# zhoupengwei/tloam

Hardware: AMD Instinct MI355X
Metric: gauss_newton_iters_per_sec (higher is better)
Workload: dtype f64

## Files before the change

tloam_amd/csrc/tl_gn.hip:

```cpp
#include <stdlib.h>
#include <string.h>

#include <hip/hip_ext.h>

#include "tl_common.hpp"
#include "tl_finish.hpp"

namespace tl {

struct Acc {
  double v[27];
  double pm;
  int pe;
};

__host__ __device__ constexpr int ut(int i, int j) { return i * 6 - (i * (i - 1)) / 2 + (j - i); }

__device__ __forceinline__ double fast_rcp(double x) {
  double r = __builtin_amdgcn_rcp(x);
  return __builtin_fma(r, __builtin_fma(-x, r, 1.0), r);
}
__device__ __forceinline__ double fast_rsqrt(double x) {
  double y = __builtin_amdgcn_rsq(x);
  const double h = 0.5 * x * y;
// ... 688 lines not shown
}
__device__ __forceinline__ void load_state_words(const GnState* st, GnState* sm) {
  constexpr int kWords = (int)(sizeof(GnState) / 8);
  static_assert(kWords <= 256, "one word per thread");
  if (threadIdx.x < kWords)
    reinterpret_cast<unsigned long long*>(sm)[threadIdx.x] = reinterpret_cast<const unsigned long long*>(st)[threadIdx.x];
}
__device__ __forceinline__ void stop_comm_error(GnState* st) {
  if (threadIdx.x == 0) { st->done = 1; st->comm_error = 1; }
}
__device__ __forceinline__ bool mbox_receive(const MboxView& mb, unsigned long long id, double* out , int count, int lane) {
  const bool ok = mbox_gather(mb, id, out, count, lane);
  if (lane == 0) {
    mb.ctr[0] = id;
    if (!ok) mb.ctr[1] = 1ull;
  }
  return ok;
}
__global__ __launch_bounds__(64) void k_gn_step(GnState* st, const double* __restrict__ in48, unsigned long long* iter_span) {
  __shared__ double tot[kReduceBuf];
  __shared__ double scr[32];
  __shared__ GnState s_in;
  if (threadIdx.x < kReduceBuf) tot[threadIdx.x] = in48[threadIdx.x];
  load_state_lds(st, &s_in, threadIdx.x);
  __syncthreads();
  if (s_in.done) return;
  const bool first = s_in.phase == PH_ITER0;
  gn_consume(st, tot, threadIdx.x, &s_in, scr);
  if (threadIdx.x == 0) iter_span_note(iter_span, first);
}
void launch_gn_step(GnState* st, const double* in48, hipStream_t s, unsigned long long* iter_span) {
  hipLaunchKernelGGL(k_gn_step, dim3(1), dim3(64), 0, s, st, in48, iter_span);
}
__global__ __launch_bounds__(64) void k_gn_step_mbox(GnState* st, MboxView mb, unsigned long long* iter_span) {
  __shared__ double tot[kMboxSlot];
  __shared__ double scr[32];
  __shared__ GnState s_in;
  load_state_lds(st, &s_in, threadIdx.x);
  __syncthreads();
  if (s_in.done) return;
  const bool ok = mbox_receive(mb, mbox_next_id(mb), tot, kReduceBuf, threadIdx.x);
  __syncthreads();
  if (!ok) {
    stop_comm_error(st);
    return;
  }
  const bool first = s_in.phase == PH_ITER0;
  gn_consume(st, tot, threadIdx.x, &s_in, scr);
  if (threadIdx.x == 0) iter_span_note(iter_span, first);
}
void launch_gn_step_mbox(GnState* st, const MboxView& mb, hipStream_t s, unsigned long long* iter_span) {
  hipLaunchKernelGGL(k_gn_step_mbox, dim3(1), dim3(64), 0, s, st, mb, iter_span);
}
__global__ __launch_bounds__(64) void k_mbox_gather_only(double* out48, MboxView mb) {
  __shared__ double tot[kMboxSlot];
  mbox_receive(mb, mbox_next_id(mb), tot, kReduceBuf, threadIdx.x);
  if (threadIdx.x < kReduceBuf) out48[threadIdx.x] = tot[threadIdx.x];
}
void launch_mbox_gather_only(double* out48, const MboxView& mb, hipStream_t s) {
  hipLaunchKernelGGL(k_mbox_gather_only, dim3(1), dim3(64), 0, s, out48, mb);
}
__global__ __launch_bounds__(64) void k_mbox_allreduce(double* buf, int count, MboxView mb) {
  __shared__ double vals[kMboxSlot];
  const int t = threadIdx.x;
  if (t < count) vals[t] = buf[t];
  __syncthreads();
  const unsigned long long id = mbox_next_id(mb);
  mbox_post(mb, id, vals, count, t);
  mbox_receive(mb, id, vals, count, t);
  __syncthreads();
  if (t < count) buf[t] = vals[t];
}
void launch_mbox_allreduce(double* buf, int count, const MboxView& mb, hipStream_t s) {
  hipLaunchKernelGGL(k_mbox_allreduce, dim3(1), dim3(64), 0, s, buf, count, mb);
}

__global__ __launch_bounds__(kRedThreads) void k_reduce_and_step(const double* __restrict__ partials, int rows,
                                                                 GnState* __restrict__ st, unsigned long long* iter_span) {
  __shared__ double lds[8 * 33];
  __shared__ double tot[kReduceBuf];
  __shared__ GnState s_in;
#ifdef TLOAM_STEP_PROFILE
  if (threadIdx.x == 0) st->dbg[0] = (double)__builtin_readcyclecounter();
#endif
  load_state_words(st, &s_in);
#ifdef TLOAM_STEP_PROFILE
  asm volatile("s_waitcnt vmcnt(0)" ::: "memory");
  if (threadIdx.x == 0) st->dbg[7] = (double)__builtin_readcyclecounter();
#endif
  fold_rows<false, 4>(partials, rows, lds, tot);
#ifdef TLOAM_STEP_PROFILE
  if (threadIdx.x == 0) st->dbg[8] = (double)__builtin_readcyclecounter();
#endif
  if (s_in.done) return;
  const bool first = s_in.phase == PH_ITER0;
  if (threadIdx.x < 64) gn_consume(st, tot, threadIdx.x, &s_in, lds );
  if (threadIdx.x == 0) iter_span_note(iter_span, first);
#ifdef TLOAM_STEP_PROFILE
  if (threadIdx.x == 0) st->dbg[6] = (double)__builtin_readcyclecounter();
#endif
}
struct K3Step {
  int* ticket;
  unsigned long long* span;
  unsigned long long* iter_span;
  MboxView mb;
};
template <bool SINGLE, int W = 4>
__global__ __launch_bounds__(64 * W, 2) void k3_sweep_step(const double* __restrict__ seg0, int stride0, int cap0, int unused,
                                                        GnState* __restrict__ st, const int* __restrict__ seg_n,
                                                        double* __restrict__ partials, CorrView cv, K3Step fs) {
  __shared__ double red[W][32];
  __shared__ double s_grp[8 * 33];
  __shared__ double tot[kMboxSlot];
  __shared__ GnState s_in;
  SweepStamps ts;
  sweep_body<SINGLE, W, false>(seg0, stride0, cap0, (unused & 2) != 0 , false, st, seg_n, cv, red,
                               ts, [&] {
    if (fs.span && blockIdx.x == 0 && threadIdx.x == 0)
      __hip_atomic_store(fs.span, (unsigned long long)wall_clock64(), __ATOMIC_RELAXED, __HIP_MEMORY_SCOPE_AGENT);
    load_state_words(st, &s_in);
  }, [&] {
    if (!k3_take_ticket<W>(partials, red, fs.ticket)) return;
    if (fs.span && threadIdx.x == 0) {
      const unsigned long long t1 = wall_clock64();
      const unsigned long long t0 = __hip_atomic_load(fs.span, __ATOMIC_RELAXED, __HIP_MEMORY_SCOPE_AGENT);
      fs.span[1] += t1 - t0;
      fs.span[2] += 1ull;
    }
    fold_rows<true>(partials, (int)gridDim.x, s_grp, tot);
    if (threadIdx.x == 0) __hip_atomic_store(fs.ticket, 0, __ATOMIC_RELAXED, __HIP_MEMORY_SCOPE_AGENT);
    if (threadIdx.x >= 64) return;
    if (fs.mb.nranks > 0) {
      const unsigned long long id = mbox_next_id(fs.mb);
      mbox_post(fs.mb, id, tot, kReduceBuf, (int)threadIdx.x);
      const bool ok = mbox_receive(fs.mb, id, tot, kReduceBuf, (int)threadIdx.x);
      asm volatile("s_waitcnt lgkmcnt(0)" ::: "memory");
      if (!ok) {
        stop_comm_error(st);
        return;
      }
    }
    const bool first = s_in.phase == PH_ITER0;
    gn_consume(st, tot, (int)threadIdx.x, &s_in, s_grp );
    if (threadIdx.x == 0) iter_span_note(fs.iter_span, first);
  });
}
void launch_k3_step(const CorrView& cv, GnState* st, double* partials, int grid, bool single, bool wide, int* ticket, unsigned long long* span,
                    const MboxView* mb_or_null, hipStream_t s, hipEvent_t ev_start, hipEvent_t ev_stop, unsigned long long* iter_span) {
  auto kern = single ? k3_sweep_step<true> : wide ? k3_sweep_step<false, 8> : k3_sweep_step<false>;
  K3Step fs;
  memset(&fs, 0, sizeof(fs));
  fs.ticket = ticket;
  fs.span = span;
  fs.iter_span = iter_span;
  if (mb_or_null) fs.mb = *mb_or_null;
  launch_sweep(kern, grid, wide ? 512 : 256, s, ev_start, ev_stop, cv, 0, st, partials, cv, fs);
}

__global__ __launch_bounds__(256, 1) void k_sweep_step_small(const double* __restrict__ seg0, int stride0, int cap0, int tagged,
                                                             GnState* __restrict__ st, const int* __restrict__ seg_n,
                                                             double* __restrict__ partials, int* __restrict__ ticket,
                                                             CorrView cv, unsigned long long* iter_span) {
  __shared__ double red[4][32];
  __shared__ double s_grp[8 * 33];
  __shared__ double s_rows[kTaggedRows * 28];
  __shared__ double tot[kReduceBuf];
  __shared__ GnState s_in;
  const int lane = threadIdx.x & 63, wave = __builtin_amdgcn_readfirstlane(threadIdx.x >> 6);
  const int gw = blockIdx.x * 4 + wave;
#ifdef TLOAM_STEP_PROFILE
  const unsigned long long c_entry = __builtin_readcyclecounter();
#endif
  ChunkData pre;
  const SingleWork wk = single_work_of(cv, cap0, gw, lane);
  const bool w2 = (tagged & 2) != 0;
  tagged &= 1;
  single_fetch(cv, seg0, stride0, wk, pre, w2);
  {
    constexpr int kWords = (int)(sizeof(GnState) / 8);
    static_assert(kWords <= 256, "one word per thread");
    if (threadIdx.x < kWords)
      reinterpret_cast<unsigned long long*>(&s_in)[threadIdx.x] = reinterpret_cast<const unsigned long long*>(st)[threadIdx.x];
  }
  unsigned long long* const epoch = reinterpret_cast<unsigned long long*>(ticket + 2);
  const unsigned long long epoch0 = *epoch;
  if (st->done) return;
  const Rt T = st->Rt_eval;
#ifdef TLOAM_STEP_PROFILE
  asm volatile("s_waitcnt lgkmcnt(0)" ::: "memory");
  const unsigned long long c_pose = __builtin_readcyclecounter();
#endif
  Acc a;
  sweep_single(cv, seg_n, T, wk, pre, a);
#ifdef TLOAM_STEP_PROFILE
  const unsigned long long c_eval = __builtin_readcyclecounter();
#endif
  const double wtot = wave_reduce_acc(a, lane);
  if ((lane & 1) == 0) red[wave][lane >> 1] = wtot;
  __syncthreads();
#ifdef TLOAM_STEP_PROFILE
  const unsigned long long c_sweep = __builtin_readcyclecounter();
#endif
  if (tagged) {
    k3_post_row_tagged(partials, red, epoch0 + 1ull);
    if (blockIdx.x != 0 || threadIdx.x >= 64) return;
#ifdef TLOAM_STEP_PROFILE
    if (threadIdx.x == 0) {
      st->dbg[7] = (double)c_sweep; st->dbg[0] = (double)__builtin_readcyclecounter();
      st->dbg[8] = (double)c_entry; st->dbg[9] = (double)c_pose; st->dbg[10] = (double)c_eval;
    }
#endif
    const bool ok = poll_fold_tagged(partials, (int)gridDim.x, epoch0 + 1ull, s_rows, tot, (int)threadIdx.x);
    if (threadIdx.x == 0) *epoch = epoch0 + 1ull;
    if (!ok) {
      if (threadIdx.x == 0) { st->done = 1; st->comm_error = 1; }
      return;
    }
  } else {
    if (!k3_take_ticket(partials, red, ticket)) return;
#ifdef TLOAM_STEP_PROFILE
    if (threadIdx.x == 0) { st->dbg[7] = (double)c_sweep; st->dbg[0] = (double)__builtin_readcyclecounter(); }
#endif
    fold_rows<true>(partials, (int)gridDim.x, s_grp, tot);
    if (threadIdx.x == 0) __hip_atomic_store(ticket, 0, __ATOMIC_RELAXED, __HIP_MEMORY_SCOPE_AGENT);
  }
  const bool first = s_in.phase == PH_ITER0;
  if (threadIdx.x < 64) gn_consume(st, tot, threadIdx.x, &s_in, s_grp );
  if (threadIdx.x == 0) iter_span_note(iter_span, first);
#ifdef TLOAM_STEP_PROFILE
  if (threadIdx.x == 0) st->dbg[6] = (double)__builtin_readcyclecounter();
#endif
}
void launch_sweep_step_small(const CorrView& cv, GnState* st, double* partials, int* ticket, int grid, hipStream_t s,
                             unsigned long long* iter_span) {
  launch_sweep(k_sweep_step_small, grid, 256, s, nullptr, nullptr, cv, grid <= kTaggedRows ? 1 : 0 , st, partials, ticket, cv,
               iter_span);
}
#include "tl_prep.hpp"

__device__ __forceinline__ bool weight_out_of_range(const WeightParams& wp, int kind, double c) {
  if (!wp.active[kind]) return false;
  if (c == 0) return false;
  if (c >= wp.th1 || c <= wp.th2) return false;
  if (c < wp.th1 * (1.0 - 1e-9) && c > wp.th2 * (1.0 + 1e-9)) return false;
  const double w = sqrt(wp.noise_bound_sq * wp.mu * (wp.mu + 1) / c) - wp.mu;
  return !(w >= 0.0 && w <= 1.0);
}
constexpr int kExtRowBase = 512;
__device__ __forceinline__ void post_ext_segment(double* __restrict__ partials, int gw, double cs, double bad, int kind, unsigned long long tag,
                                                 int lane, int base_word = kExtRowBase) {
  if (lane >= 8) return;
  unsigned long long wd = 0ull;
  const double cs0 = rdlane(cs, 0), bad0 = rdlane(bad, 0);
  if (lane == 0) wd = (unsigned long long)__double_as_longlong(cs0);
  else if (lane == 1) wd = (unsigned long long)__double_as_longlong(bad0);
  else if (lane == 2) wd = (unsigned long long)(long long)kind;
  const unsigned long long x = xor8(lane < 7 ? seg_word(wd, lane) : 0ull);
  if (lane == 7) wd = check_mix(tag) ^ x;
  __hip_atomic_store(reinterpret_cast<unsigned long long*>(partials) + base_word + (size_t)gw * 8 + lane, wd, __ATOMIC_RELAXED,
                     __HIP_MEMORY_SCOPE_AGENT);
}
__device__ __forceinline__ bool poll_fold_ext(const double* __restrict__ partials, int nwaves, unsigned long long tag, double* s_ext ,
                                              double* fin , int lane, int base_word = kExtRowBase) {
  const bool have = lane >= 1 && lane < nwaves;
  const unsigned long long mtag = check_mix(tag);
  const unsigned long long* p = reinterpret_cast<const unsigned long long*>(partials) + base_word + (size_t)(have ? lane : 1) * 8;
  unsigned long long w[8];
  const unsigned long long t0 = wall_clock64();
  bool ok_all;
  for (unsigned spins = 1;; ++spins) {
#pragma unroll
    for (int i = 0; i < 8; ++i) w[i] = __hip_atomic_load(p + i, __ATOMIC_RELAXED, __HIP_MEMORY_SCOPE_AGENT);
    unsigned long long x = w[7];
#pragma unroll
    for (int i = 0; i < 7; ++i) x ^= seg_word(w[i], i);
    ok_all = __all((!have || x == mtag) ? 1 : 0) != 0;
    if (ok_all) break;
    if ((spins & 63u) == 0 && wall_clock64() - t0 > 100000000ull) break;
    __builtin_amdgcn_s_sleep(1);
  }
  const double cs = have ? __longlong_as_double((long long)w[0]) : 0.0;
  const double bad = have ? __longlong_as_double((long long)w[1]) : 0.0;
  const int kind = have ? (int)(long long)w[2] : -1;
  double t[5];
#pragma unroll
  for (int k = 0; k < 4; ++k) t[k] = kind == k ? cs : 0.0;
  t[4] = bad;
#pragma unroll
  for (int off = 32; off > 0; off >>= 1)
#pragma unroll
    for (int k = 0; k < 5; ++k) t[k] += __shfl_down(t[k], off, 64);
  if (lane == 0) {
#pragma unroll
    for (int k = 0; k < 5; ++k) fin[k] = t[k];
  }
  asm volatile("s_waitcnt lgkmcnt(0)" ::: "memory");
  (void)s_ext;
  return ok_all;
}

__device__ __forceinline__ int finish_by_consumer(GnState* st, GnState* sm , const SolveFinish& F, int oi,
                                                  const double* fin, const int nseg[kKinds], double* sh , int lane,
                                                  bool lead = true) {
  constexpr int kWords = (int)(offsetof(GnState, dbg) / 8);
  const OuterCtl ctl{F.cost_threshold, 1, oi == F.n_iter - 1 ? 1 : 0};
  int next = 4;
  if (!sm->done) {
    if (lane == 0) {
      sm->incomplete = OS_INCOMPLETE;
      sm->stop = 2;
      sm->run_build = sm->run_refresh = 0;
    }
  } else {
    if (lane < 16) {
      double v = 0.0;
      if (lane < 4) v = fin[lane];
      else if (lane < 8) v = (double)(lane == 4 ? nseg[0] : (lane == 5 ? nseg[1] : (lane == 6 ? nseg[2] : nseg[3])));
      else if (lane == 8) v = fin[4];
      sh[lane] = v;
      if (lead) F.sums16[lane] = v;
    }
    asm volatile("s_waitcnt lgkmcnt(0)" ::: "memory");
    publish_and_rearm(sh, sm, lane, ctl);
    asm volatile("s_waitcnt lgkmcnt(0)" ::: "memory");
    next = (sm->stop == 0 && sm->run_build == 0 && sm->run_refresh != 0 && oi + 1 < F.n_iter) ? 3 : 4;
  }
  asm volatile("s_waitcnt lgkmcnt(0)" ::: "memory");
  if (!lead) return next;
  for (int w = lane; w < kWords; w += 64) reinterpret_cast<unsigned long long*>(st)[w] = reinterpret_cast<const unsigned long long*>(sm)[w];
  mirror_wave(sm, F.hm[oi], lane, (sm->stop == 0 && next == 4) ? (int)(sm->incomplete | OS_NEEDS_HOST) : -1);
  if (sm->stop != 0)
    for (int j = oi + 1; j < F.n_iter; ++j) mirror_wave(sm, F.hm[j], lane, (int)OS_SKIPPED);
  return next;
}

constexpr int kAllRowsParity = kTaggedRows * kAccStride;
constexpr int kAllExtBase = 2 * kAllRowsParity;
constexpr int kAllExtParity = 64 * 8;
__device__ __forceinline__ bool next_is_failure(const double* s_msg) {
  asm volatile("s_waitcnt lgkmcnt(0)" ::: "memory");
  return (int)s_msg[12] == 5;
}
__global__ __launch_bounds__(256, 1) void k_solve_all(const double* __restrict__ seg0, int stride0, int cap0, int max_sweeps,
                                                      GnState* __restrict__ st, const int* __restrict__ seg_n,
                                                      double* __restrict__ partials, int* __restrict__ ticket, CorrView cv, SolvePrep prep,
                                                      int* __restrict__ seg_n_out, SolveFinish F) {
  __shared__ double red[4][32];
  __shared__ double s_scr[32];
  __shared__ double s_rows[kTaggedRows * 28];
  __shared__ double s_ext[64 * 3];
  __shared__ double s_fin[8];
  __shared__ double s_sh[16];
  __shared__ double tot[kReduceBuf];
  __shared__ double s_msg[16];
  __shared__ GnState s_in;
  const int lane = threadIdx.x & 63, wave = __builtin_amdgcn_readfirstlane(threadIdx.x >> 6);
  const int gw = blockIdx.x * 4 + wave;
  const bool stepper = wave == 0;
  const bool lead = blockIdx.x == 0;
  const bool self_prep = prep.sv.flagb != nullptr;
  const unsigned long long sabotage = ((max_sweeps >> 16) & 1) ? (1ull << 40) : 0ull;
  max_sweeps &= 0xffff;
  unsigned long long* const epoch = reinterpret_cast<unsigned long long*>(ticket + 2);
#ifdef TLOAM_STEP_PROFILE
  unsigned long long* const prof = reinterpret_cast<unsigned long long*>(partials) + 2048;
  const bool prof_c = lead && stepper && lane == 0;
  const bool prof_p = (int)blockIdx.x == (int)gridDim.x / 2 && wave == 1 && lane == 0;
#define TL_PROF(cond, slot) if (cond) prof[(slot)] = wall_clock64();
#else
#define TL_PROF(cond, slot)
#endif
  ChunkData pre;
  const SingleWork wk = single_work_of(cv, cap0, gw, lane);
  single_fetch(cv, seg0, stride0, wk, pre);
  FlagBytes fbytes;
  if (self_prep && wk.kind >= 0) load_flag_bytes(prep.sv.flagb, wk.kind, lane, fbytes);
  if (stepper) {
    constexpr int kWords = (int)(sizeof(GnState) / 8);
    for (int w = lane; w < kWords; w += 64)
      reinterpret_cast<unsigned long long*>(&s_in)[w] = reinterpret_cast<const unsigned long long*>(st)[w];
  }
  const unsigned long long tag0 = (*epoch + 1ull) << 8;
  int oi = F.first_iter;
  if (F.enabled && (st->stop != 0 || st->next_outer != oi)) return;
  const bool build = self_prep && (!prep.run_build || *prep.run_build != 0);
  const bool refresh = self_prep && !build && prep.run_refresh && *prep.run_refresh != 0;
  const bool done_at_entry = st->done != 0;
  Rt T = st->Rt_eval;
  int n_mine = 0;
  int slot[2] = {0, 0};
  int nseg[kKinds] = {0, 0, 0, 0};
  if (lead && stepper) {
    if (build) {
      FlagBytes fb[kKinds];
#pragma unroll
      for (int k = 0; k < kKinds; ++k) load_flag_bytes(prep.sv.flagb, k, lane, fb[k]);
#pragma unroll
      for (int k = 0; k < kKinds; ++k) nseg[k] = kind_set_of(prep, cv, k, lane, fb[k]).total;
      if (lane < kKinds) seg_n_out[lane] = lane == 0 ? nseg[0] : (lane == 1 ? nseg[1] : (lane == 2 ? nseg[2] : nseg[3]));
    } else {
#pragma unroll
      for (int k = 0; k < kKinds; ++k) nseg[k] = seg_n[k];
    }
  }
  if (wk.kind >= 0) {
    if (build) {
      n_mine = self_compact(prep, cv, wk, lane, fbytes, pre, slot);
    } else {
      n_mine = seg_n[wk.kind];
      if (self_prep) {
        slots_of_chunk(prep, cv, wk, n_mine, slot);
        if (refresh) self_refresh(prep, cv, wk, n_mine, slot, pre);
      }
    }
  }
  if (stepper) {
    asm volatile("s_waitcnt vmcnt(0) lgkmcnt(0)" ::: "memory");
    if (build && lane < 6) {
      s_in.x_build[lane] = s_in.x[lane];
      if (lead) st->x_build[lane] = s_in.x[lane];
    }
  }
  if (done_at_entry) return;
  TL_PROF(prof_c, 0)
  unsigned long long h = 0;
  for (;;) {
    int verdict = 2;
    double2 last_cost = double2{0.0, 0.0};
    for (int it = 0;; ++it) {
      Acc a;
      last_cost = double2{0.0, 0.0};
      sweep_single_n(cv, n_mine, T, wk, pre, a, &last_cost);
      TL_PROF(prof_p, 64 + it * 8 + 1)
      const double wtot = wave_reduce_acc(a, lane);
      if ((lane & 1) == 0) red[wave][lane >> 1] = wtot;
      __syncthreads();
      double* const rows = partials + (size_t)(h & 1ull) * kAllRowsParity;
      const int ext_base = kAllExtBase + (int)(h & 1ull) * kAllExtParity;
      k3_post_row_tagged(rows, red, tag0 | h);
      TL_PROF(prof_c, 8 + it * 8 + 0)
      if (F.have_wp) {
        double cs = last_cost.x + last_cost.y;
        double bad = 0.0;
        if (wk.kind >= 0) {
          const bool two = single_chunk_of(wk.kind) == kChunk;
          if (wk.j < n_mine && weight_out_of_range(F.wp[oi], wk.kind, last_cost.x)) bad += 1.0;
          if (two && wk.j + 1 < n_mine && weight_out_of_range(F.wp[oi], wk.kind, last_cost.y)) bad += 1.0;
        }
#pragma unroll
        for (int off = 32; off > 0; off >>= 1) {
          cs += __shfl_down(cs, off, 64);
          bad += __shfl_down(bad, off, 64);
        }
        post_ext_segment(partials, gw, cs, bad, wk.kind, tag0 | h, lane, ext_base);
      }
      TL_PROF(prof_p, 64 + it * 8 + 2)
      if (stepper) {
        const bool ok = poll_fold_tagged(rows, (int)gridDim.x, (tag0 | h) ^ sabotage, s_rows, tot, lane);
        TL_PROF(prof_c, 8 + it * 8 + 1)
        int vd = 5;
        if (ok) {
          gn_consume(st, tot, lane, &s_in, s_scr, false);
          vd = (s_in.done == 0 && it + 1 < max_sweeps) ? 1 : 2;
          if (lead && lane == 0) iter_span_note(F.iter_span, it == 0);
        }
        TL_PROF(prof_c, 8 + it * 8 + 2)
        if (lane < 9) s_msg[lane] = s_in.Rt_eval.r[lane];
        else if (lane < 12) s_msg[lane] = s_in.Rt_eval.t[lane - 9];
        else if (lane == 12) s_msg[12] = (double)vd;
      }
      __syncthreads();
      verdict = (int)s_msg[12];
      if (lead && stepper && verdict != 5) gn_write_back(st, &s_in, lane);
#pragma unroll
      for (int v = 0; v < 9; ++v) T.r[v] = s_msg[v];
#pragma unroll
      for (int v = 0; v < 3; ++v) T.t[v] = s_msg[9 + v];
      TL_PROF(prof_c, 8 + it * 8 + 3)
      TL_PROF(prof_p, 64 + (it + 1) * 8 + 0)
      h += 1ull;
      if (verdict != 1) break;
    }
    if (verdict == 5) {
      if (lead && stepper) {
        if (lane == 0) {
          st->done = 1; st->comm_error = 1;
          s_in.done = 1; s_in.comm_error = 1;
          if (F.enabled) {
            s_in.incomplete = OS_COMM_ERROR;
            st->incomplete = OS_COMM_ERROR;
            st->stop = 1; st->run_build = 0; st->run_refresh = 0;
          }
          *epoch = tag0 >> 8;
        }
        asm volatile("s_waitcnt lgkmcnt(0)" ::: "memory");
        if (F.enabled) {
          mirror_wave(&s_in, F.hm[oi], lane, (int)OS_COMM_ERROR);
          for (int j = oi + 1; j < F.n_iter; ++j) mirror_wave(&s_in, F.hm[j], lane, (int)OS_SKIPPED);
        }
      }
      return;
    }
    double2 w_new = pre.w;
    if (F.enabled && wk.kind >= 0) {
      const bool two = single_chunk_of(wk.kind) == kChunk;
      if (wk.j < n_mine) w_new.x = refreshed_weight(F.wp[oi], wk.kind, last_cost.x, pre.w.x, prep.sv.w_src, slot[0]);
      if (two && wk.j + 1 < n_mine) w_new.y = refreshed_weight(F.wp[oi], wk.kind, last_cost.y, pre.w.y, prep.sv.w_src, slot[1]);
    }
    if (stepper) {
      int next = 4;
      bool ok = true;
      if (F.have_wp)
        ok = poll_fold_ext(partials, (int)gridDim.x * 4, tag0 | (h - 1ull), s_ext, s_fin, lane, kAllExtBase + (int)((h - 1ull) & 1ull) * kAllExtParity);
      if (!ok) {
        next = 5;
      } else if (!F.enabled) {
        if (lead) {
          if (F.have_wp && lane < 5) {
            const double v = s_fin[lane];
            if (lane < 4) st->fin_sum[lane] = v; else st->fin_bad = v;
          }
          if (lane == 0) { st->fin_valid = F.have_wp ? 1 : 0; *epoch = tag0 >> 8; }
        }
      } else {
        next = finish_by_consumer(st, &s_in, F, oi, s_fin, nseg, s_sh, lane, lead);
      }
      if (lane < 9) s_msg[lane] = s_in.Rt_eval.r[lane];
      else if (lane < 12) s_msg[lane] = s_in.Rt_eval.t[lane - 9];
      else if (lane == 12) s_msg[12] = (double)next;
    }
    if (!F.enabled) {
      if (lead && stepper && next_is_failure(s_msg) && lane == 0) {
        st->done = 1; st->comm_error = 1; s_in.done = 1; s_in.comm_error = 1;
        st->fin_valid = 0;
        *epoch = tag0 >> 8;
      }
      return;
    }
    __syncthreads();
    const int next = (int)s_msg[12];
#pragma unroll
    for (int v = 0; v < 9; ++v) T.r[v] = s_msg[v];
#pragma unroll
    for (int v = 0; v < 3; ++v) T.t[v] = s_msg[9 + v];
    if (next == 5) {
      if (lead && stepper) {
        if (lane == 0) {
          st->done = 1; st->comm_error = 1; s_in.done = 1; s_in.comm_error = 1;
          s_in.incomplete = OS_COMM_ERROR; st->incomplete = OS_COMM_ERROR;
          st->stop = 1; st->run_build = 0; st->run_refresh = 0;
          *epoch = tag0 >> 8;
        }
        asm volatile("s_waitcnt lgkmcnt(0)" ::: "memory");
        mirror_wave(&s_in, F.hm[oi], lane, (int)OS_COMM_ERROR);
        for (int j = oi + 1; j < F.n_iter; ++j) mirror_wave(&s_in, F.hm[j], lane, (int)OS_SKIPPED);
      }
      return;
    }
    if (next != 3) {
      if (lead && stepper && lane == 0) *epoch = tag0 >> 8;
      return;
    }
    if (wk.kind >= 0) {
      const CorrSeg& seg = cv.k[wk.kind];
      const bool two = single_chunk_of(wk.kind) == kChunk;
      pre.w = w_new;
      if (wk.j < n_mine) { seg.w[wk.j] = w_new.x; seg.cost[wk.j] = 0.0; }
      if (two && wk.j + 1 < n_mine) { seg.w[wk.j + 1] = w_new.y; seg.cost[wk.j + 1] = 0.0; }
    }
    oi += 1;
  }
}
void launch_solve_small(const CorrView& cv, GnState* st, double* partials, int* ticket, int grid, int max_sweeps,
                        const SolvePrep* prep_or_null, int* seg_n, const SolveFinish* finish_or_null, hipStream_t s) {
  SolvePrep P;
  if (prep_or_null) P = *prep_or_null;
  else memset(&P, 0, sizeof(P));
  SolveFinish F;
  if (finish_or_null) F = *finish_or_null;
  else memset(&F, 0, sizeof(F));
  hipLaunchKernelGGL(k_solve_all, dim3(grid), dim3(256), 0, s, (const double*)cv.k[0].px, cv.k[0].stride, cv.k[0].cap, max_sweeps, st,
                     cv.seg_n, partials, ticket, cv, P, seg_n, F);
}
bool solve_small_fits(int grid, int device_cus) { return grid <= kTaggedRows && grid <= device_cus; }
void launch_reduce_and_step(const double* partials, int grid, GnState* st, hipStream_t s, unsigned long long* iter_span) {
  hipLaunchKernelGGL(k_reduce_and_step, dim3(1), dim3(kRedThreads), 0, s, partials, grid, st, iter_span);
}

__global__ void k_debug_se3(const double* __restrict__ x, const double* __restrict__ delta, int n, double* __restrict__ out) {
  const int i = blockIdx.x * blockDim.x + threadIdx.x;
  if (i >= n) return;
  double xv[6], dv[6];
#pragma unroll
  for (int k = 0; k < 6; ++k) { xv[k] = x[6 * i + k]; dv[k] = delta[6 * i + k]; }
  const Pose E = exp_fast2(dv);
  const Pose X = exp_fast2(xv);
  double lx[6], pl[6];
  log_fast2(X, lx);
  log_fast2(compose_fast2(E, X), pl);
  const Pose X2 = se3_exp(xv);
  double* o = out + 26 * (size_t)i;
  o[0] = E.qw; o[1] = E.qx; o[2] = E.qy; o[3] = E.qz; o[4] = E.tx; o[5] = E.ty; o[6] = E.tz;
#pragma unroll
  for (int k = 0; k < 6; ++k) { o[7 + k] = lx[k]; o[13 + k] = pl[k]; }
  o[19] = X2.qw; o[20] = X2.qx; o[21] = X2.qy; o[22] = X2.qz; o[23] = X2.tx; o[24] = X2.ty; o[25] = X2.tz;
}
void launch_debug_se3(const double* x, const double* delta, int n, double* out, hipStream_t s) {
  hipLaunchKernelGGL(k_debug_se3, dim3((n + 63) / 64), dim3(64), 0, s, x, delta, n, out);
}

__global__ __launch_bounds__(256) void k_weights(WeightArgs A, double* __restrict__ partial, const GnState* __restrict__ st) {
  __shared__ double red[4][8];
  if (!st->done || st->stop) return;
  double sum[kKinds] = {0, 0, 0, 0};
  double bad = 0.0;
  const int tid = blockIdx.x * 256 + threadIdx.x, stride = gridDim.x * 256;
#pragma unroll
  for (int k = 0; k < kKinds; ++k) {
    const int n = A.cv.seg_n[k];
    const CorrSeg& seg = A.cv.k[k];
    constexpr int kU = 4;
    for (int i0 = tid; i0 < n; i0 += kU * stride) {
      double cu[kU];
      int iu[kU];
#pragma unroll
      for (int u = 0; u < kU; ++u) {
        const int i = i0 + u * stride;
        cu[u] = (i < n) ? seg.cost[i] : 0.0;
        iu[u] = (i < n) ? seg.idx[i] : 0;
      }
#pragma unroll
      for (int u = 0; u < kU; ++u) {
        if (i0 + u * stride >= n) break;
        const double c = cu[u];
        sum[k] += c;
        if (!A.wp.active[k]) continue;
        if (c == 0) continue;
        double w;
        if (c >= A.wp.th1) w = 0.0;
        else if (c <= A.wp.th2) w = 1.0;
        else {
          w = sqrt(A.wp.noise_bound_sq * A.wp.mu * (A.wp.mu + 1) / c) - A.wp.mu;
          if (!(w >= 0.0 && w <= 1.0)) bad += 1.0;
        }
        const int slot = A.sv.slot_off[k] + (iu[u] - A.sv.src_lo[k]);
        A.sv.w_src[slot] = w;
      }
    }
  }
  double v[5] = {sum[0], sum[1], sum[2], sum[3], bad};
  const int lane = threadIdx.x & 63, wave = threadIdx.x >> 6;
#pragma unroll
  for (int i = 0; i < 5; ++i) {
#pragma unroll
    for (int off = 32; off > 0; off >>= 1) v[i] += __shfl_down(v[i], off, 64);
    if (lane == 0) red[wave][i] = v[i];
  }
  __syncthreads();
  if (threadIdx.x < 8) {
    double t = 0.0;
    if (threadIdx.x < 5) t = ((red[0][threadIdx.x] + red[1][threadIdx.x]) + red[2][threadIdx.x]) + red[3][threadIdx.x];
    partial[blockIdx.x * 8 + threadIdx.x] = t;
  }
}
void launch_weights(const CorrView& cv, const SlotView& sv, const WeightParams& wp, double* partial, int blocks,
                    const GnState* st, hipStream_t s) {
  WeightArgs A;
  A.cv = cv;
  A.sv = sv;
  A.wp = wp;
  hipLaunchKernelGGL(k_weights, dim3(blocks), dim3(256), 0, s, A, partial, st);
}

__global__ __launch_bounds__(64) void k_outer_finish(const double* __restrict__ partial, int blocks,
                                                     const int* __restrict__ seg_n, double* __restrict__ sums16,
                                                     GnState* st_or_null, GnState* gate, HostMirror hm, OuterCtl ctl) {
  __shared__ double sh[16];
  const int t = threadIdx.x;
  {
    const int g = finish_gate(gate, ctl, t);
    if (g != 0) {
      if (st_or_null) mirror_to_host(gate, hm, t, 64, g == 1 ? (int)OS_SKIPPED : -1);
      return;
    }
  }
  double v[5] = {0, 0, 0, 0, 0};
  for (int b = t; b < blocks; b += 64) {
#pragma unroll
    for (int c = 0; c < 5; ++c) v[c] += partial[b * 8 + c];
  }
#pragma unroll
  for (int c = 0; c < 5; ++c)
#pragma unroll
    for (int off = 32; off > 0; off >>= 1) v[c] += __shfl_down(v[c], off, 64);
  if (t < 16) sh[t] = 0.0;
  __syncthreads();
  if (t == 0) {
#pragma unroll
    for (int c = 0; c < 4; ++c) sh[c] = v[c];
    sh[8] = v[4];
  }
  if (t >= 4 && t < 8) sh[t] = (double)seg_n[t - 4];
  __syncthreads();
  if (t < 16) sums16[t] = sh[t];
  if (st_or_null) {
    publish_and_rearm(sh, st_or_null, t, ctl);
    mirror_to_host(st_or_null, hm, t, 64);
  }
}
void launch_outer_finish(const double* partial, int blocks, const int* seg_n, GnState* st_or_null, GnState* gate,
                         double* sums16, HostMirror hm, OuterCtl ctl, hipStream_t s) {
  hipLaunchKernelGGL(k_outer_finish, dim3(1), dim3(64), 0, s, partial, blocks, seg_n, sums16, st_or_null, gate, hm, ctl);
}
__global__ void k_outer_publish(const double* __restrict__ sums16, GnState* st, HostMirror hm,
                                const unsigned long long* __restrict__ comm_err) {
  if (st->done) publish_and_rearm(sums16, st, threadIdx.x, OuterCtl{0.0, 0, 0});
  if (threadIdx.x == 0 && (st->comm_error || (comm_err && *comm_err))) st->incomplete = 3;
  mirror_to_host(st, hm, threadIdx.x, 64);
}
void launch_outer_publish(const double* sums16, GnState* st, HostMirror hm, const unsigned long long* comm_err,
                          hipStream_t s) {
  hipLaunchKernelGGL(k_outer_publish, dim3(1), dim3(64), 0, s, sums16, st, hm, comm_err);
}

struct Mat16 { double m[16]; };
__global__ void k_transform(double* aos, size_t n, Mat16 M) {
  size_t i = (size_t)blockIdx.x * blockDim.x + threadIdx.x;
  const size_t stride = (size_t)gridDim.x * blockDim.x;
  for (; i < n; i += stride) {
    const double x = aos[3 * i], y = aos[3 * i + 1], z = aos[3 * i + 2];
    double o[4];
#pragma unroll
    for (int r = 0; r < 4; ++r) o[r] = M.m[r] * x + M.m[4 + r] * y + M.m[8 + r] * z + M.m[12 + r];
    aos[3 * i] = o[0] / o[3];
    aos[3 * i + 1] = o[1] / o[3];
    aos[3 * i + 2] = o[2] / o[3];
  }
}
void launch_transform_cloud(double* aos, size_t n, const double M[16], hipStream_t s) {
  if (n == 0) return;
  Mat16 m;
  for (int i = 0; i < 16; ++i) m.m[i] = M[i];
  int blocks = (int)((n + 255) / 256);
  if (blocks > 4096) blocks = 4096;
  hipLaunchKernelGGL(k_transform, dim3(blocks), dim3(256), 0, s, aos, n, m);
}

}
```

Before: 61920.

## Overlap external-sum fold on wave 1 and defer state write-out past broadcast

In block 0, the fold of the weight/cost external partials moves off the stepper wave and onto wave 1. Wave 1 starts it after the stepper has folded the tagged rows, signalled through a shared-memory counter, so it overlaps with gn_consume. Copying state back to global memory and mirroring to host now happen after the block-wide broadcast, which takes them off the path the other waves wait on. Profiling probes are also extended, but they only compile under a debug macro. The cost is an extra spin-wait on a shared counter and more LDS synchronisation, which carries some ordering risk.

```diff
diff --git a/tloam_amd/csrc/tl_gn.hip b/tloam_amd/csrc/tl_gn.hip
--- a/tloam_amd/csrc/tl_gn.hip
+++ b/tloam_amd/csrc/tl_gn.hip
@@ -1014,8 +1014,7 @@
 
 __device__ __forceinline__ int finish_by_consumer(GnState* st, GnState* sm , const SolveFinish& F, int oi,
                                                   const double* fin, const int nseg[kKinds], double* sh , int lane,
-                                                  bool lead = true) {
-  constexpr int kWords = (int)(offsetof(GnState, dbg) / 8);
+                                                  bool lead = true, unsigned long long* prof_published = nullptr) {
   const OuterCtl ctl{F.cost_threshold, 1, oi == F.n_iter - 1 ? 1 : 0};
   int next = 4;
   if (!sm->done) {
@@ -1036,15 +1035,23 @@
     asm volatile("s_waitcnt lgkmcnt(0)" ::: "memory");
     publish_and_rearm(sh, sm, lane, ctl);
     asm volatile("s_waitcnt lgkmcnt(0)" ::: "memory");
+#ifdef TLOAM_STEP_PROFILE
+    if (prof_published && lane == 0) *prof_published = wall_clock64();
+#else
+    (void)prof_published;
+#endif
     next = (sm->stop == 0 && sm->run_build == 0 && sm->run_refresh != 0 && oi + 1 < F.n_iter) ? 3 : 4;
   }
   asm volatile("s_waitcnt lgkmcnt(0)" ::: "memory");
-  if (!lead) return next;
+  return next;
+}
+__device__ __forceinline__ void finish_write_out(GnState* st, const GnState* sm , const SolveFinish& F, int oi, int next,
+                                                 int lane) {
+  constexpr int kWords = (int)(offsetof(GnState, dbg) / 8);
   for (int w = lane; w < kWords; w += 64) reinterpret_cast<unsigned long long*>(st)[w] = reinterpret_cast<const unsigned long long*>(sm)[w];
   mirror_wave(sm, F.hm[oi], lane, (sm->stop == 0 && next == 4) ? (int)(sm->incomplete | OS_NEEDS_HOST) : -1);
   if (sm->stop != 0)
     for (int j = oi + 1; j < F.n_iter; ++j) mirror_wave(sm, F.hm[j], lane, (int)OS_SKIPPED);
-  return next;
 }
 
 constexpr int kAllRowsParity = kTaggedRows * kAccStride;
@@ -1067,6 +1074,7 @@
   __shared__ double tot[kReduceBuf];
   __shared__ double s_msg[16];
   __shared__ GnState s_in;
+  __shared__ unsigned s_rows_in;
   const int lane = threadIdx.x & 63, wave = __builtin_amdgcn_readfirstlane(threadIdx.x >> 6);
   const int gw = blockIdx.x * 4 + wave;
   const bool stepper = wave == 0;
@@ -1076,13 +1084,15 @@
   max_sweeps &= 0xffff;
   unsigned long long* const epoch = reinterpret_cast<unsigned long long*>(ticket + 2);
 #ifdef TLOAM_STEP_PROFILE
-  unsigned long long* const prof = reinterpret_cast<unsigned long long*>(partials) + 2048;
+  unsigned long long* const prof = reinterpret_cast<unsigned long long*>(partials) + 2048 + (F.first_iter & 1) * 1024;
   const bool prof_c = lead && stepper && lane == 0;
   const bool prof_p = (int)blockIdx.x == (int)gridDim.x / 2 && wave == 1 && lane == 0;
 #define TL_PROF(cond, slot) if (cond) prof[(slot)] = wall_clock64();
 #else
 #define TL_PROF(cond, slot)
 #endif
+  TL_PROF(prof_c, 1)
+  TL_PROF(prof_p, 8)
   ChunkData pre;
   const SingleWork wk = single_work_of(cv, cap0, gw, lane);
   single_fetch(cv, seg0, stride0, wk, pre);
@@ -1096,6 +1106,8 @@
   const unsigned long long tag0 = (*epoch + 1ull) << 8;
   int oi = F.first_iter;
   if (F.enabled && (st->stop != 0 || st->next_outer != oi)) return;
+  TL_PROF(prof_c, 2)
+  TL_PROF(prof_p, 9)
   const bool build = self_prep && (!prep.run_build || *prep.run_build != 0);
   const bool refresh = self_prep && !build && prep.run_refresh && *prep.run_refresh != 0;
   const bool done_at_entry = st->done != 0;
@@ -1115,6 +1127,7 @@
 #pragma unroll
       for (int k = 0; k < kKinds; ++k) nseg[k] = seg_n[k];
     }
+    TL_PROF(prof_c, 3)
   }
   if (wk.kind >= 0) {
     if (build) {
@@ -1127,15 +1140,32 @@
       }
     }
   }
+  TL_PROF(prof_p, 10)
+#ifdef TLOAM_STEP_PROFILE
+  if (prof_p) {
+    asm volatile("s_waitcnt vmcnt(0)" ::: "memory");
+    prof[11] = wall_clock64();
+  }
+#endif
   if (stepper) {
     asm volatile("s_waitcnt vmcnt(0) lgkmcnt(0)" ::: "memory");
     if (build && lane < 6) {
       s_in.x_build[lane] = s_in.x[lane];
       if (lead) st->x_build[lane] = s_in.x[lane];
     }
+    TL_PROF(prof_c, 5)
   }
   if (done_at_entry) return;
+  if (threadIdx.x == 0) s_rows_in = 0u;
   TL_PROF(prof_c, 0)
+#ifdef TLOAM_STEP_PROFILE
+  const int q0 = oi;
+#define TL_PROF_H(cond, base, k) if (cond && h < 24ull) prof[(base) + 4 * (int)h + (k)] = wall_clock64();
+#define TL_PROF_Q(cond, k) if (cond && oi - q0 < 4) prof[208 + 16 * (oi - q0) + (k)] = wall_clock64();
+#else
+#define TL_PROF_H(cond, base, k)
+#define TL_PROF_Q(cond, k)
+#endif
   unsigned long long h = 0;
   for (;;) {
     int verdict = 2;
@@ -1144,14 +1174,14 @@
       Acc a;
       last_cost = double2{0.0, 0.0};
       sweep_single_n(cv, n_mine, T, wk, pre, a, &last_cost);
-      TL_PROF(prof_p, 64 + it * 8 + 1)
+      TL_PROF_H(prof_p, 112, 1)
       const double wtot = wave_reduce_acc(a, lane);
       if ((lane & 1) == 0) red[wave][lane >> 1] = wtot;
       __syncthreads();
       double* const rows = partials + (size_t)(h & 1ull) * kAllRowsParity;
       const int ext_base = kAllExtBase + (int)(h & 1ull) * kAllExtParity;
       k3_post_row_tagged(rows, red, tag0 | h);
-      TL_PROF(prof_c, 8 + it * 8 + 0)
+      TL_PROF_H(prof_c, 16, 0)
       if (F.have_wp) {
         double cs = last_cost.x + last_cost.y;
         double bad = 0.0;
@@ -1167,17 +1197,23 @@
         }
         post_ext_segment(partials, gw, cs, bad, wk.kind, tag0 | h, lane, ext_base);
       }
-      TL_PROF(prof_p, 64 + it * 8 + 2)
+      TL_PROF_H(prof_p, 112, 2)
+      if (F.have_wp && wave == 1) {
+        while (__hip_atomic_load(&s_rows_in, __ATOMIC_RELAXED, __HIP_MEMORY_SCOPE_WORKGROUP) != (unsigned)h + 1u) __builtin_amdgcn_s_sleep(2);
+        const bool ok = poll_fold_ext(partials, (int)gridDim.x * 4, tag0 | h, s_ext, s_fin, lane, ext_base);
+        if (lane == 0) s_fin[5] = ok ? 1.0 : 0.0;
+      }
       if (stepper) {
         const bool ok = poll_fold_tagged(rows, (int)gridDim.x, (tag0 | h) ^ sabotage, s_rows, tot, lane);
-        TL_PROF(prof_c, 8 + it * 8 + 1)
+        if (lane == 0) __hip_atomic_store(&s_rows_in, (unsigned)h + 1u, __ATOMIC_RELAXED, __HIP_MEMORY_SCOPE_WORKGROUP);
+        TL_PROF_H(prof_c, 16, 1)
         int vd = 5;
         if (ok) {
           gn_consume(st, tot, lane, &s_in, s_scr, false);
           vd = (s_in.done == 0 && it + 1 < max_sweeps) ? 1 : 2;
           if (lead && lane == 0) iter_span_note(F.iter_span, it == 0);
         }
-        TL_PROF(prof_c, 8 + it * 8 + 2)
+        TL_PROF_H(prof_c, 16, 2)
         if (lane < 9) s_msg[lane] = s_in.Rt_eval.r[lane];
         else if (lane < 12) s_msg[lane] = s_in.Rt_eval.t[lane - 9];
         else if (lane == 12) s_msg[12] = (double)vd;
@@ -1189,9 +1225,9 @@
       for (int v = 0; v < 9; ++v) T.r[v] = s_msg[v];
 #pragma unroll
       for (int v = 0; v < 3; ++v) T.t[v] = s_msg[9 + v];
-      TL_PROF(prof_c, 8 + it * 8 + 3)
-      TL_PROF(prof_p, 64 + (it + 1) * 8 + 0)
+      TL_PROF_H(prof_c, 16, 3)
       h += 1ull;
+      TL_PROF_H(prof_p, 112, 0)
       if (verdict != 1) break;
     }
     if (verdict == 5) {
@@ -1214,17 +1250,21 @@
       }
       return;
     }
+    TL_PROF_Q(prof_c, 0)
+    TL_PROF_Q(prof_p, 8)
     double2 w_new = pre.w;
     if (F.enabled && wk.kind >= 0) {
       const bool two = single_chunk_of(wk.kind) == kChunk;
       if (wk.j < n_mine) w_new.x = refreshed_weight(F.wp[oi], wk.kind, last_cost.x, pre.w.x, prep.sv.w_src, slot[0]);
       if (two && wk.j + 1 < n_mine) w_new.y = refreshed_weight(F.wp[oi], wk.kind, last_cost.y, pre.w.y, prep.sv.w_src, slot[1]);
     }
+    TL_PROF_Q(prof_c, 1)
+    TL_PROF_Q(prof_p, 9)
     if (stepper) {
       int next = 4;
       bool ok = true;
-      if (F.have_wp)
-        ok = poll_fold_ext(partials, (int)gridDim.x * 4, tag0 | (h - 1ull), s_ext, s_fin, lane, kAllExtBase + (int)((h - 1ull) & 1ull) * kAllExtParity);
+      if (F.have_wp) ok = s_fin[5] != 0.0;
+      TL_PROF_Q(prof_c, 2)
       if (!ok) {
         next = 5;
       } else if (!F.enabled) {
@@ -1236,7 +1276,13 @@
           if (lane == 0) { st->fin_valid = F.have_wp ? 1 : 0; *epoch = tag0 >> 8; }
         }
       } else {
+#ifdef TLOAM_STEP_PROFILE
+        next = finish_by_consumer(st, &s_in, F, oi, s_fin, nseg, s_sh, lane, lead,
+                                  prof_c && oi - q0 < 4 ? prof + 208 + 16 * (oi - q0) + 3 : nullptr);
+#else
         next = finish_by_consumer(st, &s_in, F, oi, s_fin, nseg, s_sh, lane, lead);
+#endif
+        TL_PROF_Q(prof_c, 4)
       }
       if (lane < 9) s_msg[lane] = s_in.Rt_eval.r[lane];
       else if (lane < 12) s_msg[lane] = s_in.Rt_eval.t[lane - 9];
@@ -1252,6 +1298,8 @@
     }
     __syncthreads();
     const int next = (int)s_msg[12];
+    TL_PROF_Q(prof_c, 5)
+    TL_PROF_Q(prof_p, 10)
 #pragma unroll
     for (int v = 0; v < 9; ++v) T.r[v] = s_msg[v];
 #pragma unroll
@@ -1270,8 +1318,11 @@
       }
       return;
     }
+    if (lead && stepper) finish_write_out(st, &s_in, F, oi, next, lane);
     if (next != 3) {
       if (lead && stepper && lane == 0) *epoch = tag0 >> 8;
+      TL_PROF_Q(prof_c, 6)
+      TL_PROF_Q(prof_p, 11)
       return;
     }
     if (wk.kind >= 0) {
@@ -1281,8 +1332,12 @@
       if (wk.j < n_mine) { seg.w[wk.j] = w_new.x; seg.cost[wk.j] = 0.0; }
       if (two && wk.j + 1 < n_mine) { seg.w[wk.j + 1] = w_new.y; seg.cost[wk.j + 1] = 0.0; }
     }
+    TL_PROF_Q(prof_c, 6)
+    TL_PROF_Q(prof_p, 11)
     oi += 1;
   }
+#undef TL_PROF_H
+#undef TL_PROF_Q
 }
 void launch_solve_small(const CorrView& cv, GnState* st, double* partials, int* ticket, int grid, int max_sweeps,
                         const SolvePrep* prep_or_null, int* seg_n, const SolveFinish* finish_or_null, hipStream_t s) {
```

Result: faster. 63360 (median of 6 runs) (+2.3%).
